# dusk-network/dusk-blindbidproof

Hardware: AMD Instinct MI355X
Metric: blind-bid proofs/sec (higher is better)
Workload: dtype u32

## Files before the change

### dusk_blindbidproof_amd/csrc/msm.hip

```cpp
#include "context.h"

namespace bbp {

#ifndef BBP_FOLD_PRIO
#define BBP_FOLD_PRIO 2
#endif
#ifndef BBP_MSM_WAVES
#define BBP_MSM_WAVES 2
#endif
#ifndef BBP_MSM_WAVES_MAX
#define BBP_MSM_WAVES_MAX 2
#endif

#ifdef BBP_MSM_PROF
__device__ unsigned long long g_msm_prof[8];
#define MSM_PROF_BEGIN() unsigned long long prof_t = wall_clock64()
#define MSM_PROF_MARK(i)                                                    \
    if (tid == 0) {                                                         \
        unsigned long long now_ = wall_clock64();                           \
        atomicAdd(&g_msm_prof[i], now_ - prof_t);                           \
        prof_t = now_;                                                      \
    }
#else
#define MSM_PROF_BEGIN()
// ... 11 lines not shown

__device__ __forceinline__ void xch_put(u32* xch, const ge& p) {
    const u32* w = reinterpret_cast<const u32*>(&p);
#pragma unroll
    for (int i = 0; i < GE_WORDS; i++) xch[i] = w[i];
}

__device__ __forceinline__ ge xch_get(const u32* xch) {
    ge p;
    u32* w = reinterpret_cast<u32*>(&p);
#pragma unroll
    for (int i = 0; i < GE_WORDS; i++) w[i] = xch[i];
    return p;
}

__device__ __forceinline__ row_regs load_row(const niels_row* __restrict__ tab, u32 entry, u32* __restrict__ fault) {
    u32 row = entry & 0x7fffffffu;
    if (row > (u32)(TAB_BASES * MSM_POS - 1)) {
        row = (u32)(TAB_BASES * MSM_POS - 1);
        atomicOr(fault, 1u);
    }
#ifdef BBP_EXP_ROWMASK
    row &= BBP_EXP_ROWMASK;
#endif
    return load_row_at(tab + row, entry >> 31);
}

#ifdef BBP_ACC_COOP
constexpr int COOP_IMG = 64 * 128;
__device__ __forceinline__ u32 coop_clamp_row(u32 entry, u32* __restrict__ fault) {
    u32 row = entry & 0x7fffffffu;
    if (row > (u32)(TAB_BASES * MSM_POS - 1)) {
        row = (u32)(TAB_BASES * MSM_POS - 1);
        atomicOr(fault, 1u);
    }
    return row;
}
__device__ __forceinline__ void coop_issue(const niels_row* __restrict__ tab, u8* wb, u32 my_row, int lane, u32 srcoff) {
    const u8* t = reinterpret_cast<const u8*>(tab);
    u32 r[8];
#pragma unroll
    for (int j = 0; j < 8; j++) r[j] = (u32)__shfl((int)my_row, 8 * j + (lane >> 3), 64);
#pragma unroll
    for (int j = 0; j < 8; j++) {
        const u8* src = t + (size_t)r[j] * 128 + (srcoff ^ (u32)((j & 1) << 6));
        __builtin_amdgcn_global_load_lds((const __attribute__((address_space(1))) void*)src, (__attribute__((address_space(3))) void*)(wb + j * 1024), 16, 0, 0);
    }
}
__device__ __forceinline__ row_regs coop_read(const u8* wb, u32 A, u32 neg) {
    const u32 An = A ^ (neg << 6);
    const uint4 a0 = *reinterpret_cast<const uint4*>(wb + An), a1 = *reinterpret_cast<const uint4*>(wb + (An ^ 0x10u));
    const uint2 a2 = *reinterpret_cast<const uint2*>(wb + (An ^ 0x20u));
    const uint4 b0 = *reinterpret_cast<const uint4*>(wb + (An ^ 0x40u)), b1 = *reinterpret_cast<const uint4*>(wb + (An ^ 0x50u));
    const uint2 b2 = *reinterpret_cast<const uint2*>(wb + (An ^ 0x60u));
    const uint2 x0 = *reinterpret_cast<const uint2*>(wb + (A ^ 0x20u) + 8);
    const uint4 x1 = *reinterpret_cast<const uint4*>(wb + (A ^ 0x30u));
    const uint2 x2 = *reinterpret_cast<const uint2*>(wb + (A ^ 0x60u) + 8), x3 = *reinterpret_cast<const uint2*>(wb + (A ^ 0x70u));
    row_regs r;
    r.ypx = fe{{(i32)a0.x, (i32)a0.y, (i32)a0.z, (i32)a0.w, (i32)a1.x, (i32)a1.y, (i32)a1.z, (i32)a1.w, (i32)a2.x, (i32)a2.y}};
    r.ymx = fe{{(i32)b0.x, (i32)b0.y, (i32)b0.z, (i32)b0.w, (i32)b1.x, (i32)b1.y, (i32)b1.z, (i32)b1.w, (i32)b2.x, (i32)b2.y}};
    r.xy2d = fe{{(i32)x0.x, (i32)x0.y, (i32)x1.x, (i32)x1.y, (i32)x1.z, (i32)x1.w, (i32)x2.x, (i32)x2.y, (i32)x3.x, (i32)x3.y}};
    return r;
}
#endif

__device__ __noinline__ void ge_add_nc(ge& r, const ge& a, const ge& b) { r = ge_add(a, b); }
__device__ __noinline__ void ge_dbl_nc(ge& r, const ge& a) { r = ge_dbl(a); }

#ifndef BBP_SORT_T
#define BBP_SORT_T 1024
#endif
constexpr int SORT_T = BBP_SORT_T;
template <int MODE> struct msm_geom;
template <> struct msm_geom<0> { static constexpr int K = MSM_K, NAF = MSM_NAF, W = MSM_W; };
template <> struct msm_geom<1> { static constexpr int K = FOLD_K, NAF = FOLD_NAF, W = FOLD_W; };
template <> struct msm_geom<2> { static constexpr int K = SMALL_K, NAF = SMALL_NAF, W = SMALL_W; };

template <int MODE>
__global__ __launch_bounds__(SORT_T) void k_msm_sort(const u32* __restrict__ scal_a, const u32* __restrict__ aux, u32 n_total, u32 n_idx_sets,
                                                      u32 n_sub, u32 split, u32* __restrict__ sorted_all, u32* __restrict__ cursor_all,
                                                      const u32* __restrict__ msm_map, const u32* __restrict__ n_active, u32* __restrict__ ticket) {
    constexpr int K = msm_geom<MODE>::K, NAF = msm_geom<MODE>::NAF, W = msm_geom<MODE>::W, G = K >= SORT_T ? K / SORT_T : 1;
    __shared__ u32 cursor[K + 1];
    __shared__ u32 part[SORT_T];
    const int tid = threadIdx.x;
    if (ticket && blockIdx.x == 0 && tid == 0) *ticket = 0;
    if (n_active && blockIdx.x >= *n_active) return;
    const size_t work = blockIdx.x, msm = work / split;
    const u32 i0 = (u32)(work % split) * n_sub;
    const u32 n = i0 < n_total ? min(n_sub, n_total - i0) : 0u;
    __builtin_amdgcn_s_setprio(3);
    const u32* sbase;
    const u32* base_idx = nullptr;
    u32 base0 = 0;
    if (MODE != 1) {
        const size_t src = msm_map ? (size_t)msm_map[msm] : msm;
        sbase = scal_a + (src * (size_t)n_total + i0) * 8;
        base_idx = aux + (size_t)(msm % n_idx_sets) * n_total + i0;
    } else {
        const u32 side = (u32)msm & 1u;
        sbase = (side ? aux : scal_a) + ((msm >> 1) * (size_t)2048 + i0) * 8;
        base0 = (side ? BBP_BASE_H0 : BBP_BASE_G0) + i0;
    }
    u32* sorted = sorted_all + work * (size_t)n_sub * W;
    auto key = [&](u32 i, u32 mag) -> u32 { return (MODE != 1 ? 0u : ((i0 + i) & (FOLD_CLS - 1)) * FOLD_M) + ((mag + 1) >> 1); };

    for (int k = tid; k <= K; k += SORT_T) cursor[k] = 0;
    __syncthreads();
    for (u32 i = tid; i < n; i += SORT_T) {
        const uint4* sp = reinterpret_cast<const uint4*>(sbase + (size_t)i * 8);
        uint4 lo = sp[0], hi = sp[1];
        const u32 s[8] = {lo.x, lo.y, lo.z, lo.w, hi.x, hi.y, hi.z, hi.w};
        if (MODE != 1 && base_idx[i] == MSM_SKIP_BASE) continue;
        sc_for_each_naf_digit<NAF>(s, [&](u32, u32 mag, u32) { atomicAdd(&cursor[key(i, mag)], 1u); });
    }
    __syncthreads();
    {
        u32 local = 0;
        for (int r = 1; r <= G; r++)
            if (tid * G + r <= K) local += cursor[tid * G + r];
        const int lane = tid & 63, wave = tid >> 6;
        u32 incl = local;
#pragma unroll
        for (int d = 1; d < 64; d <<= 1) {
            const u32 up = (u32)__shfl_up((int)incl, d, 64);
            if (lane >= d) incl += up;
        }
        if (lane == 63) part[wave] = incl;
        __syncthreads();
        if (tid < 64) {
            constexpr int NW = SORT_T / 64;
            u32 v = tid < NW ? part[tid] : 0u, sc_ = v;
#pragma unroll
            for (int d = 1; d < 64; d <<= 1) {
                const u32 up = (u32)__shfl_up((int)sc_, d, 64);
                if (tid >= d) sc_ += up;
            }
            if (tid < NW) part[tid] = sc_ - v;
        }
        __syncthreads();
        u32 base = part[wave] + incl - local;
        for (int r = 1; r <= G; r++) {
            if (tid * G + r > K) break;
            const u32 c = cursor[tid * G + r];
            cursor[tid * G + r] = base;
            base += c;
        }
    }
    __syncthreads();
    for (u32 i = tid; i < n; i += SORT_T) {
        const uint4* sp = reinterpret_cast<const uint4*>(sbase + (size_t)i * 8);
        uint4 lo = sp[0], hi = sp[1];
        const u32 s[8] = {lo.x, lo.y, lo.z, lo.w, hi.x, hi.y, hi.z, hi.w};
        if (MODE != 1 && base_idx[i] == MSM_SKIP_BASE) continue;
        const u32 tb = (MODE != 1 ? base_idx[i] : base0 + i) * MSM_POS;
        sc_for_each_naf_digit<NAF>(s, [&](u32 pos, u32 mag, u32 neg) {
            u32 at = atomicAdd(&cursor[key(i, mag)], 1u);
            sorted[at] = (tb + pos) | (neg << 31);
        });
    }
    __syncthreads();
    u32* cur_out = cursor_all + work * (size_t)(K + 1);
    for (int k = tid; k <= K; k += SORT_T) cur_out[k] = k ? cursor[k] : 0u;
}

#ifndef BBP_SORT_CAP
#define BBP_SORT_CAP 21504
#endif
template <int MODE> struct sort_cap { static constexpr u32 V = BBP_SORT_CAP; };
template <> struct sort_cap<1> { static constexpr u32 V = 8192; };
constexpr u32 SORT_CAP_WIDE = 32768;
constexpr u32 SORT_WIDE_FROM = 3000;

template <int MODE>
__global__ __launch_bounds__(SORT_T) void k_msm_sort_staged(const u32* __restrict__ scal_a, const u32* __restrict__ aux, u32 n_total, u32 n_idx_sets,
                                                             u32 n_sub, u32 split, u32* __restrict__ sorted_all, u32* __restrict__ cursor_all,
                                                             const u32* __restrict__ msm_map, const u32* __restrict__ n_active, u32 CAP, u32* __restrict__ ticket) {
    constexpr int K = msm_geom<MODE>::K, NAF = msm_geom<MODE>::NAF, W = msm_geom<MODE>::W, G = K >= SORT_T ? K / SORT_T : 1;
    extern __shared__ u32 stage[];
    __shared__ u32 start[K + 2];
    __shared__ u32 fill[K + 1];
    __shared__ u32 part[SORT_T];
    const int tid = threadIdx.x;
    if (ticket && blockIdx.x == 0 && tid == 0) *ticket = 0;
    if (n_active && blockIdx.x >= *n_active) return;
    const size_t work = blockIdx.x, msm = work / split;
    const u32 i0 = (u32)(work % split) * n_sub;
    const u32 n = i0 < n_total ? min(n_sub, n_total - i0) : 0u;
    __builtin_amdgcn_s_setprio(3);
    const u32* sbase;
    const u32* base_idx = nullptr;
    u32 base0 = 0;
    if (MODE != 1) {
        const size_t src = msm_map ? (size_t)msm_map[msm] : msm;
        sbase = scal_a + (src * (size_t)n_total + i0) * 8;
        base_idx = aux + (size_t)(msm % n_idx_sets) * n_total + i0;
    } else {
        const u32 side = (u32)msm & 1u;
        sbase = (side ? aux : scal_a) + ((msm >> 1) * (size_t)2048 + i0) * 8;
        base0 = (side ? BBP_BASE_H0 : BBP_BASE_G0) + i0;
    }
    u32* sorted = sorted_all + work * (size_t)n_sub * W;
    auto key = [&](u32 i, u32 mag) -> u32 { return (MODE != 1 ? 0u : ((i0 + i) & (FOLD_CLS - 1)) * FOLD_M) + ((mag + 1) >> 1); };

    for (int k = tid; k <= K; k += SORT_T) fill[k] = 0;
    __syncthreads();
    for (u32 i = tid; i < n; i += SORT_T) {
        const uint4* sp = reinterpret_cast<const uint4*>(sbase + (size_t)i * 8);
        uint4 lo = sp[0], hi = sp[1];
        const u32 s[8] = {lo.x, lo.y, lo.z, lo.w, hi.x, hi.y, hi.z, hi.w};
        if (MODE != 1 && base_idx[i] == MSM_SKIP_BASE) continue;
        sc_for_each_naf_digit<NAF>(s, [&](u32, u32 mag, u32) { atomicAdd(&fill[key(i, mag)], 1u); });
    }
    __syncthreads();
    {
        u32 local = 0;
        for (int r = 1; r <= G; r++)
            if (tid * G + r <= K) local += fill[tid * G + r];
        const int lane = tid & 63, wave = tid >> 6;
        u32 incl = local;
#pragma unroll
        for (int d = 1; d < 64; d <<= 1) {
            const u32 up = (u32)__shfl_up((int)incl, d, 64);
            if (lane >= d) incl += up;
        }
        if (lane == 63) part[wave] = incl;
        __syncthreads();
        if (tid < 64) {
            constexpr int NW = SORT_T / 64;
            u32 v = tid < NW ? part[tid] : 0u, sc_ = v;
#pragma unroll
            for (int d = 1; d < 64; d <<= 1) {
                const u32 up = (u32)__shfl_up((int)sc_, d, 64);
                if (tid >= d) sc_ += up;
            }
            if (tid < NW) part[tid] = sc_ - v;
        }
        __syncthreads();
        u32 base = part[wave] + incl - local;
        for (int r = 1; r <= G; r++) {
            if (tid * G + r > K) break;
            const u32 c = fill[tid * G + r];
            start[tid * G + r] = base;
            fill[tid * G + r] = 0;
            base += c;
        }
        if (tid == SORT_T - 1) start[K + 1] = base;
        if (tid == 0) start[0] = 0;
    }
    __syncthreads();
    u32 kb = 1;
    while (kb <= (u32)K) {
        const u32 base = start[kb];
        const bool direct = start[kb + 1] - base > CAP;
        u32 ke = kb + 1;
        if (!direct) {
            u32 lo = kb + 1, hi = (u32)K + 1;
            while (lo < hi) {
                const u32 mid = (lo + hi + 1) >> 1;
                if (start[mid] - base <= CAP) lo = mid; else hi = mid - 1;
            }
            ke = lo;
        }
        if (start[ke] != base) {
            for (u32 i = tid; i < n; i += SORT_T) {
                const uint4* sp = reinterpret_cast<const uint4*>(sbase + (size_t)i * 8);
                uint4 lo4 = sp[0], hi4 = sp[1];
                const u32 s[8] = {lo4.x, lo4.y, lo4.z, lo4.w, hi4.x, hi4.y, hi4.z, hi4.w};
                if (MODE != 1 && base_idx[i] == MSM_SKIP_BASE) continue;
                const u32 tb = (MODE != 1 ? base_idx[i] : base0 + i) * MSM_POS;
                sc_for_each_naf_digit<NAF>(s, [&](u32 pos, u32 mag, u32 neg) {
                    const u32 k = key(i, mag);
                    if (k >= kb && k < ke) {
                        const u32 at = start[k] + atomicAdd(&fill[k], 1u);
                        const u32 ent = (tb + pos) | (neg << 31);
                        if (direct) sorted[at] = ent; else stage[at - base] = ent;
                    }
                });
            }
            __syncthreads();
            if (!direct) {
                const u32 cnt = start[ke] - base;
                for (u32 i = tid; i < cnt; i += SORT_T) sorted[base + i] = stage[i];
            }
            __syncthreads();
        }
        kb = ke;
    }
    u32* cur_out = cursor_all + work * (size_t)(K + 1);
    for (int k = tid; k <= K; k += SORT_T) cur_out[k] = k ? start[k + 1] : 0u;
}

#ifndef BBP_ACC_WG
#define BBP_ACC_WG 256
#endif
constexpr int ACC_WG = BBP_ACC_WG, ACC_WGS = ACC_T / ACC_WG;
static_assert(ACC_T % ACC_WG == 0 && ACC_WG % 64 == 0, "accumulate workgroup geometry");

template <int MODE>
__global__ __launch_bounds__(ACC_WG) __attribute__((amdgpu_waves_per_eu(BBP_MSM_WAVES, BBP_MSM_WAVES_MAX)))
void k_msm_acc(const niels_row* __restrict__ ptable, const u32* __restrict__ sorted_all, const u32* __restrict__ cursor_all, u32 n ,
               ge* __restrict__ bsum_all, ge* __restrict__ psum_all, ge* __restrict__ out, const u32* __restrict__ n_active, u32* __restrict__ fault,
               u32 n_work, u32* __restrict__ ticket) {
    constexpr int K = msm_geom<MODE>::K, W = msm_geom<MODE>::W, G = K / MSM_T;
    __shared__ u32 cursor[K + 1];
#ifdef BBP_ACC_PERSIST
    static_assert(ACC_WGS == 1, "the persistent form draws whole MSMs");
    __shared__ u32 s_ticket;
  for (;;) {
    __syncthreads();
    if (threadIdx.x == 0) s_ticket = atomicAdd(ticket, 1u);
    __syncthreads();
    const size_t msm = s_ticket;
    if (msm >= n_work || (n_active && msm >= *n_active)) return;
    const int tid = (int)threadIdx.x;
#else
    const size_t msm = blockIdx.x / ACC_WGS;
    const int tid = (int)(blockIdx.x % ACC_WGS) * ACC_WG + (int)threadIdx.x;
    if (n_active && msm >= *n_active) return;
#endif
    const u32* sorted = sorted_all + msm * (size_t)n * W;
#ifdef BBP_MSM_PRIO
    __builtin_amdgcn_s_setprio(BBP_MSM_PRIO);
#endif
    MSM_PROF_BEGIN();
    {
        const u32* cur_in = cursor_all + msm * (size_t)(K + 1);
        for (int k = threadIdx.x; k <= K; k += ACC_WG) cursor[k] = cur_in[k];
    }
    __syncthreads();
    MSM_PROF_MARK(1);

    const u32 E = cursor[K];
    ge* bsum = bsum_all + msm * (size_t)K;
    ge* psum = psum_all + msm * (size_t)ACC_T;
#ifdef BBP_KO_ACC_PERMILLE
    const u32 c0 = (u32)(((u64)tid * E) / ACC_T), c1 = c0 + (u32)(((u64)((u32)(((u64)(tid + 1) * E) / ACC_T) - c0) * BBP_KO_ACC_PERMILLE) / 1000);
#else
    const u32 c0 = (u32)(((u64)tid * E) / ACC_T), c1 = (u32)(((u64)(tid + 1) * E) / ACC_T);
#endif
#ifdef BBP_MSM_PROF
    const unsigned long long clk0 = clock64();
#endif
    u32 k_first = 0;
    bool inside = false;
#ifdef BBP_ACC_COOP
    {
        __shared__ __attribute__((aligned(1024))) u8 rowimg[ACC_WG / 64][COOP_IMG];
        const int lane = (int)threadIdx.x & 63;
        u8* wb = rowimg[threadIdx.x >> 6];
        const u32 A = (u32)lane * 128u + ((((u32)lane >> 1) & 7u) << 4);
        const u32 srcoff = (((u32)lane & 7u) ^ (((u32)lane >> 3) >> 1)) << 4;
        const u32 n_it = (E + (u32)ACC_T - 1) / (u32)ACC_T, len = c1 - c0;
        u32 k = 1, kend = 0;
        ge* dest = &psum[tid];
        if (len) {
            u32 lo = 1, hi = K;
            while (lo < hi) {
                u32 mid = (lo + hi) >> 1;
                if (cursor[mid] > c0) hi = mid; else lo = mid + 1;
            }
            k = lo, kend = cursor[k];
            k_first = lo;
            inside = cursor[k - 1] < c0;
            if (!inside) dest = &bsum[k - 1];
        }
        ge acc = ge_identity();
        u32 ent_cur = len ? sorted[c0] : 0u;
        u32 ent_nxt = len > 1 ? sorted[c0 + 1] : 0u;
        if (n_it) coop_issue(ptable, wb, coop_clamp_row(ent_cur, fault), lane, srcoff);
        for (u32 it = 0; it < n_it; it++) {
            const u32 e = c0 + it;
            const row_regs cur = coop_read(wb, A, ent_cur >> 31);
            const bool neg = ent_cur >> 31;
            ent_cur = ent_nxt;
            const bool live = it < len;
            if (live && e == kend) {
                *dest = acc;
                acc = ge_identity();
                do { k++; kend = cursor[k]; } while (kend == e);
                dest = &bsum[k - 1];
            }
            asm volatile("s_waitcnt lgkmcnt(0)" ::: "memory");
            if (it + 1 < n_it) coop_issue(ptable, wb, coop_clamp_row(ent_cur, fault), lane, srcoff);
            if (it + 2 < len) ent_nxt = sorted[e + 2]; else ent_nxt = 0u;
            if (live) acc = ge_madd_row(acc, cur, neg);
        }
        if (len) *dest = acc;
    }
#else
    if (c0 < c1) {
        u32 lo = 1, hi = K;
        while (lo < hi) {
            u32 mid = (lo + hi) >> 1;
            if (cursor[mid] > c0) hi = mid; else lo = mid + 1;
        }
        u32 k = lo, kend = cursor[k];
        k_first = lo;
        inside = cursor[k - 1] < c0;
        ge* dest = inside ? &psum[tid] : &bsum[k - 1];
        ge acc = ge_identity();
        u32 ent_cur = sorted[c0];
        u32 ent_nxt = (c0 + 1 < c1) ? sorted[c0 + 1] : 0u;
        row_regs row = load_row(ptable, ent_cur, fault);
        for (u32 e = c0; e < c1; e++) {
            if (e == kend) {
                *dest = acc;
                acc = ge_identity();
                do { k++; kend = cursor[k]; } while (kend == e);
                dest = &bsum[k - 1];
            }
            const row_regs cur = row;
            const bool neg = ent_cur >> 31;
            ent_cur = ent_nxt;
            if (e + 1 < c1) row = load_row(ptable, ent_cur, fault);
            if (e + 2 < c1) ent_nxt = sorted[e + 2];
            acc = ge_madd_row(acc, cur, neg);
        }
        *dest = acc;
    }
#endif
#ifdef BBP_MSM_PROF
    if (tid == 0) atomicAdd(&g_msm_prof[6], clock64() - clk0);
#endif
    MSM_PROF_MARK(2);
    __threadfence_block();
    __syncthreads();
    MSM_PROF_MARK(3);
#ifdef BBP_ACC_PERSIST
  }
#endif
}

template <int MODE>
__global__ __launch_bounds__(MSM_T) void k_msm_fold(const u32* __restrict__ cursor_all, ge* __restrict__ bsum_all, const ge* __restrict__ psum_all,
                                                     ge* __restrict__ out, const u32* __restrict__ n_active) {
    constexpr int K = msm_geom<MODE>::K, G = K / MSM_T;
    __shared__ u32 cursor[K + 1];
    __shared__ u32 xch[GE_WORDS];
    const int tid = threadIdx.x;
    if (n_active && blockIdx.x >= *n_active) return;
    __builtin_amdgcn_s_setprio(BBP_FOLD_PRIO);
    const size_t msm = blockIdx.x;
    {
        const u32* cur_in = cursor_all + msm * (size_t)(K + 1);
        for (int k = tid; k <= K; k += MSM_T) cursor[k] = cur_in[k];
// ... 292 lines not shown
    }
    if (o < n_out && j == 0) out[o] = acc;
}

static u32 msm_split(u32 n_msm, u32 n_terms) {
    static const u32 below = [] { const char* e = getenv("BBP_MSM_SPLIT_BELOW"); return e ? (u32)atoi(e) : 128u; }();
    static const u32 target = [] { const char* e = getenv("BBP_MSM_SPLIT_TARGET"); return e ? (u32)atoi(e) : 512u; }();
    if (n_msm >= below) return 1;
    u32 s = target / n_msm;
    if (s > 16) s = 16;
    while (s > 1 && n_terms / s < 128) s--;
    return s ? s : 1;
}

struct MsmScratch {
    u32 *sorted, *cursor;
    ge *bsum, *psum, *tmp;
    u32* ticket;
    size_t bytes;
};
static MsmScratch msm_scratch_layout(void* base, size_t n_msm, size_t n_terms, size_t W, size_t K, size_t out_items = 1) {
    auto up = [](size_t x) { return (x + 255) / 256 * 256; };
    MsmScratch m;
    size_t o = 0;
    m.sorted = reinterpret_cast<u32*>(static_cast<u8*>(base) + o);
    o += up(n_msm * n_terms * W * sizeof(u32));
    m.cursor = reinterpret_cast<u32*>(static_cast<u8*>(base) + o);
    o += up(n_msm * (K + 1) * sizeof(u32));
    m.bsum = reinterpret_cast<ge*>(static_cast<u8*>(base) + o);
    o += n_msm * K * sizeof(ge);
    m.psum = reinterpret_cast<ge*>(static_cast<u8*>(base) + o);
    o += n_msm * ACC_T * sizeof(ge);
    m.tmp = reinterpret_cast<ge*>(static_cast<u8*>(base) + o);
    o += up(n_msm * out_items * sizeof(ge));
    m.ticket = reinterpret_cast<u32*>(static_cast<u8*>(base) + o);
    o += 256;
    m.bytes = o;
    return m;
}
size_t msm_scratch_bytes(uint32_t n_msm, uint32_t n_terms) {
    const u32 split = msm_split(n_msm, n_terms), n_sub = (n_terms + split - 1) / split;
    size_t a = msm_scratch_layout(nullptr, (size_t)n_msm * split, n_sub, MSM_W, MSM_K).bytes;
    if (split > 1) a = std::max(a, msm_scratch_layout(nullptr, (size_t)n_msm * split, n_sub, SMALL_W, SMALL_K).bytes);
    const size_t b = msm_scratch_layout(nullptr, n_msm, n_terms, MSM_W, MSM_K).bytes;
    return a > b ? a : b;
}

static inline u32 acc_grid(bbp_ctx*, u32 n_work) {
#ifdef BBP_ACC_PERSIST
    static const u32 cap = [] { const char* e = getenv("BBP_ACC_PERSIST_GRID"); return e ? (u32)atoi(e) : 512u; }();
    return n_work < cap ? n_work : cap;
#else
    return n_work * ACC_WGS;
#endif
}

int32_t fold_generators_launch(bbp_ctx* ctx, uint32_t n_proofs, const sc* g_dev, const sc* h_dev, ge* out_dev, hipStream_t stream,
                               int scratch_slot) {
    if (n_proofs == 0) return BBP_OK;
    const size_t n_msm = 2 * (size_t)n_proofs;
    const u32 split = msm_split((u32)n_msm, 2048), n_sub = (2048 + split - 1) / split;
    const size_t n_work = n_msm * split;
    DevBuf& scratch = ctx->slice_fold[scratch_slot];
    int32_t rc = dev_reserve(ctx, scratch, msm_scratch_layout(nullptr, n_work, n_sub, FOLD_W, FOLD_K, FOLD_CLS).bytes);
    if (rc) return rc;
    const MsmScratch m = msm_scratch_layout(scratch.p, n_work, n_sub, FOLD_W, FOLD_K, FOLD_CLS);
    {
        ScopedEvent ev(ctx, TAG_MSM_SORT, stream);
        if (ctx->sort_staged & 2) {
            if (!ctx->sort_lds_attr1) {
                BBP_HIP_TRY(ctx, hipFuncSetAttribute((const void*)k_msm_sort_staged<1>, hipFuncAttributeMaxDynamicSharedMemorySize, (int)(sort_cap<1>::V * 4)));
                ctx->sort_lds_attr1 = true;
            }
            hipLaunchKernelGGL(k_msm_sort_staged<1>, dim3((u32)n_work), dim3(SORT_T), sort_cap<1>::V * 4, stream, (const u32*)g_dev, (const u32*)h_dev, 2048u, 1u,
                               n_sub, split, m.sorted, m.cursor, (const u32*)nullptr, (const u32*)nullptr, sort_cap<1>::V, m.ticket);
        } else
            hipLaunchKernelGGL(k_msm_sort<1>, dim3((u32)n_work), dim3(SORT_T), 0, stream, (const u32*)g_dev, (const u32*)h_dev, 2048u, 1u, n_sub, split,
                               m.sorted, m.cursor, (const u32*)nullptr, (const u32*)nullptr, m.ticket);
        BBP_HIP_TRY(ctx, hipGetLastError());
    }
    {
        ScopedEvent ev(ctx, TAG_MSM, stream);
        hipLaunchKernelGGL(k_msm_acc<1>, dim3(acc_grid(ctx, (u32)n_work)), dim3(ACC_WG), 0, stream, ctx->ptable, m.sorted, m.cursor, n_sub, m.bsum, m.psum,
                           split > 1 ? m.tmp : out_dev, (const u32*)nullptr, ctx->health, (u32)n_work, m.ticket);
        BBP_HIP_TRY(ctx, hipGetLastError());
    }
    ScopedEvent evf(ctx, TAG_MSM_FOLD, stream);
    hipLaunchKernelGGL(k_msm_fold<1>, dim3((u32)n_work), dim3(MSM_T), 0, stream, m.cursor, m.bsum, m.psum, split > 1 ? m.tmp : out_dev,
                       (const u32*)nullptr);
    BBP_HIP_TRY(ctx, hipGetLastError());
    if (split > 1) {
        const u32 n_out = (u32)n_msm * FOLD_CLS;
        hipLaunchKernelGGL(k_msm_reduce, dim3((n_out * REDUCE_L + 63) / 64), dim3(64), lds_token(ctx), stream, n_out, split, (u32)FOLD_CLS, m.tmp, out_dev);
        BBP_HIP_TRY(ctx, hipGetLastError());
    }
    return BBP_OK;
}

__global__ __launch_bounds__(64) void k_encode(const ge* __restrict__ pts, u32 n, u32* __restrict__ out_words) {
// ... 15 lines not shown
    if (n_msm == 0) return BBP_OK;
    if (n_terms == 0 || n_terms > 65535u) {
        ctx->err = "msm_launch: n_terms out of range";
        return BBP_ERR_BAD_ARG;
    }
    DevBuf& scratch = scratch_slot ? ctx->slice_sorted[scratch_slot] : ctx->sorted;
    int32_t rc = dev_reserve(ctx, scratch, msm_scratch_bytes(n_msm, n_terms));
    if (rc) return rc;
    const u32 split = n_active_dev ? 1u : msm_split(n_msm, n_terms), n_sub = (n_terms + split - 1) / split;
    const u32 n_work = n_msm * split;
    if (split > 1 && ctx->msm_small) {
        const MsmScratch ms = msm_scratch_layout(scratch.p, n_work, n_sub, SMALL_W, SMALL_K);
        {
            ScopedEvent ev(ctx, TAG_MSM_SORT, stream);
            hipLaunchKernelGGL(k_msm_sort<2>, dim3(n_work), dim3(SORT_T), 0, stream, scalars_dev, base_idx_dev, n_terms, n_idx_sets, n_sub, split, ms.sorted, ms.cursor,
                               msm_map_dev, n_active_dev, ms.ticket);
            BBP_HIP_TRY(ctx, hipGetLastError());
        }
        if (ctx->debug_corrupt) {
            ctx->debug_corrupt = 0;
            hipLaunchKernelGGL(k_debug_poke, dim3(1), dim3(1), 0, stream, ms.sorted);
            BBP_HIP_TRY(ctx, hipGetLastError());
        }
        {
            ScopedEvent ev(ctx, TAG_MSM, stream);
            hipLaunchKernelGGL(k_msm_acc<2>, dim3(acc_grid(ctx, n_work)), dim3(ACC_WG), 0, stream, ctx->ptable, ms.sorted, ms.cursor, n_sub, ms.bsum, ms.psum, ms.tmp,
                               n_active_dev, ctx->health, n_work, ms.ticket);
            BBP_HIP_TRY(ctx, hipGetLastError());
        }
        {
            ScopedEvent evf(ctx, TAG_MSM_FOLD, stream);
            hipLaunchKernelGGL(k_msm_fold<2>, dim3(n_work), dim3(MSM_T), 0, stream, ms.cursor, ms.bsum, ms.psum, ms.tmp, n_active_dev);
            BBP_HIP_TRY(ctx, hipGetLastError());
        }
        hipLaunchKernelGGL(k_msm_reduce, dim3((n_msm * REDUCE_L + 63) / 64), dim3(64), lds_token(ctx), stream, n_msm, split, 1u, ms.tmp, out_points_dev);
        BBP_HIP_TRY(ctx, hipGetLastError());
        return BBP_OK;
    }
    const MsmScratch m = msm_scratch_layout(scratch.p, n_work, n_sub, MSM_W, MSM_K);
    {
        ScopedEvent ev(ctx, TAG_MSM_SORT, stream);
        const bool wide = n_sub > SORT_WIDE_FROM;
        if ((ctx->sort_staged & 1) && (!wide || (ctx->sort_staged & 4))) {
            const u32 cap = wide ? SORT_CAP_WIDE : sort_cap<0>::V;
            if (!ctx->sort_lds_attr) {
                BBP_HIP_TRY(ctx, hipFuncSetAttribute((const void*)k_msm_sort_staged<0>, hipFuncAttributeMaxDynamicSharedMemorySize, (int)(SORT_CAP_WIDE * 4)));
                ctx->sort_lds_attr = true;
            }
            hipLaunchKernelGGL(k_msm_sort_staged<0>, dim3(n_work), dim3(SORT_T), cap * 4, stream, scalars_dev, base_idx_dev, n_terms, n_idx_sets, n_sub, split,
                               m.sorted, m.cursor, msm_map_dev, n_active_dev, cap, m.ticket);
        }
        else
            hipLaunchKernelGGL(k_msm_sort<0>, dim3(n_work), dim3(SORT_T), 0, stream, scalars_dev, base_idx_dev, n_terms, n_idx_sets, n_sub, split,
                               m.sorted, m.cursor, msm_map_dev, n_active_dev, m.ticket);
        BBP_HIP_TRY(ctx, hipGetLastError());
    }
    if (ctx->debug_corrupt) {
        ctx->debug_corrupt = 0;
        hipLaunchKernelGGL(k_debug_poke, dim3(1), dim3(1), 0, stream, m.sorted);
        BBP_HIP_TRY(ctx, hipGetLastError());
    }
    chain_acc = chain_acc && ctx->verify_serial_acc;
    if (chain_acc && ctx->vacc_valid)
        BBP_HIP_TRY(ctx, hipStreamWaitEvent(stream, ctx->ev_vacc[ctx->vacc_seq % bbp_ctx::VACC_RING], 0));
    {
        ScopedEvent ev(ctx, TAG_MSM, stream);
        hipLaunchKernelGGL(k_msm_acc<0>, dim3(acc_grid(ctx, n_work)), dim3(ACC_WG), 0, stream, ctx->ptable, m.sorted, m.cursor, n_sub, m.bsum, m.psum,
                           split > 1 ? m.tmp : out_points_dev, n_active_dev, ctx->health, n_work, m.ticket);
        BBP_HIP_TRY(ctx, hipGetLastError());
    }
    static const bool chain_after_fold = getenv("BBP_VERIFY_CHAIN_AFTER_FOLD") && atoi(getenv("BBP_VERIFY_CHAIN_AFTER_FOLD"));
    if (chain_acc && !chain_after_fold) {
        ctx->vacc_seq++;
        BBP_HIP_TRY(ctx, hipEventRecord(ctx->ev_vacc[ctx->vacc_seq % bbp_ctx::VACC_RING], stream));
        ctx->vacc_valid = true;
    }
    ScopedEvent evf(ctx, TAG_MSM_FOLD, stream);
    if (n_work >= (u32)ctx->fold_half_from)
        hipLaunchKernelGGL(k_msm_fold_half, dim3((n_work + 1) / 2), dim3(64), 0, stream, m.cursor, m.bsum, m.psum, split > 1 ? m.tmp : out_points_dev,
                           n_work, n_active_dev);
    else
        hipLaunchKernelGGL(k_msm_fold<0>, dim3(n_work), dim3(MSM_T), 0, stream, m.cursor, m.bsum, m.psum, split > 1 ? m.tmp : out_points_dev, n_active_dev);
    BBP_HIP_TRY(ctx, hipGetLastError());
// ... 32 lines not shown
```

### dusk_blindbidproof_amd/csrc/point.h

```cpp
#pragma once
#include "field.h"

namespace bbp {

struct ge {
    fe X, Y, Z, T;
};

struct ge_niels {
    fe ypx, ymx, xy2d;
};

struct niels_packed {
    u32 w[24];
};

struct alignas(128) niels_row {
    i32 v[32];
};

BBP_HD niels_packed niels_pack(const ge_niels& n) {
    niels_packed p;
    fe_towords(p.w, n.ypx);
    fe_towords(p.w + 8, n.ymx);
// ... 133 lines not shown
}

__device__ __forceinline__ ge ge_madd_row(const ge& p, const row_regs& q, bool neg) {
    fe a = fe_mul(fe_sub(p.Y, p.X), q.ymx);
    fe b = fe_mul(fe_add(p.Y, p.X), q.ypx);
    fe c = fe_mul(p.T, q.xy2d);
    fe d = fe_add(p.Z, p.Z);
    fe e = fe_sub(b, a), h = fe_add(b, a);
    fe f0 = fe_sub(d, c), g0 = fe_add(d, c);
    fe f = fe_select(f0, g0, neg), g = fe_select(g0, f0, neg);
    ge r;
    r.X = fe_mul(e, f);
    r.Y = fe_mul(g, h);
    r.Z = fe_mul(g, f);
    r.T = fe_mul(e, h);
    return r;
}
#endif

BBP_HD ge_niels ge_to_niels(const ge& p, const fe& zinv) {
    fe x = fe_mul(p.X, zinv), y = fe_mul(p.Y, zinv);
    ge_niels r;
    r.ypx = fe_add(y, x);
    r.ymx = fe_sub(y, x);
    r.xy2d = fe_mul(fe_mul(x, y), fe_d2());
    return r;
}

BBP_HD ge ge_from_niels(const ge_niels& n) {
    const fe half = BBP_FE_LIT(0xfffffff7u, 0xffffffffu, 0xffffffffu, 0xffffffffu, 0xffffffffu, 0xffffffffu, 0xffffffffu, 0x3fffffffu);
// ... 96 lines not shown
```

Before: 21450.

## Split MSM buckets by sign so accumulation skips per-point negation

The sort kernels now bucket entries by sign as well as magnitude and emit a per-bucket boundary (cpos) between the negative and positive runs. The accumulation kernel adds the negative run first, negates the partial sum once, then continues with the positives. This removes the per-entry conditional negation from the mixed-add inner loop. Row loads become plain 8x uint4 loads with an asm wait anchor and a sched_barrier in the madd. The unused cooperative-LDS and persistent-ticket paths are dropped, and the extra scratch array costs more memory traffic in the sort.

```diff
diff --git a/dusk_blindbidproof_amd/csrc/msm.hip b/dusk_blindbidproof_amd/csrc/msm.hip
--- a/dusk_blindbidproof_amd/csrc/msm.hip
+++ b/dusk_blindbidproof_amd/csrc/msm.hip
@@ -49,8 +49,11 @@
     return p;
 }
 
-__device__ __forceinline__ row_regs load_row(const niels_row* __restrict__ tab, u32 entry, u32* __restrict__ fault) {
-    u32 row = entry & 0x7fffffffu;
+struct row_fetch {
+    row_regs r;
+    u32 pad0, pad1;
+};
+__device__ __forceinline__ row_fetch load_row(const niels_row* __restrict__ tab, u32 row, u32* __restrict__ fault) {
     if (row > (u32)(TAB_BASES * MSM_POS - 1)) {
         row = (u32)(TAB_BASES * MSM_POS - 1);
         atomicOr(fault, 1u);
@@ -58,46 +61,16 @@
 #ifdef BBP_EXP_ROWMASK
     row &= BBP_EXP_ROWMASK;
 #endif
-    return load_row_at(tab + row, entry >> 31);
-}
-
-#ifdef BBP_ACC_COOP
-constexpr int COOP_IMG = 64 * 128;
-__device__ __forceinline__ u32 coop_clamp_row(u32 entry, u32* __restrict__ fault) {
-    u32 row = entry & 0x7fffffffu;
-    if (row > (u32)(TAB_BASES * MSM_POS - 1)) {
-        row = (u32)(TAB_BASES * MSM_POS - 1);
-        atomicOr(fault, 1u);
-    }
-    return row;
-}
-__device__ __forceinline__ void coop_issue(const niels_row* __restrict__ tab, u8* wb, u32 my_row, int lane, u32 srcoff) {
-    const u8* t = reinterpret_cast<const u8*>(tab);
-    u32 r[8];
-#pragma unroll
-    for (int j = 0; j < 8; j++) r[j] = (u32)__shfl((int)my_row, 8 * j + (lane >> 3), 64);
-#pragma unroll
-    for (int j = 0; j < 8; j++) {
-        const u8* src = t + (size_t)r[j] * 128 + (srcoff ^ (u32)((j & 1) << 6));
-        __builtin_amdgcn_global_load_lds((const __attribute__((address_space(1))) void*)src, (__attribute__((address_space(3))) void*)(wb + j * 1024), 16, 0, 0);
-    }
-}
-__device__ __forceinline__ row_regs coop_read(const u8* wb, u32 A, u32 neg) {
-    const u32 An = A ^ (neg << 6);
-    const uint4 a0 = *reinterpret_cast<const uint4*>(wb + An), a1 = *reinterpret_cast<const uint4*>(wb + (An ^ 0x10u));
-    const uint2 a2 = *reinterpret_cast<const uint2*>(wb + (An ^ 0x20u));
-    const uint4 b0 = *reinterpret_cast<const uint4*>(wb + (An ^ 0x40u)), b1 = *reinterpret_cast<const uint4*>(wb + (An ^ 0x50u));
-    const uint2 b2 = *reinterpret_cast<const uint2*>(wb + (An ^ 0x60u));
-    const uint2 x0 = *reinterpret_cast<const uint2*>(wb + (A ^ 0x20u) + 8);
-    const uint4 x1 = *reinterpret_cast<const uint4*>(wb + (A ^ 0x30u));
-    const uint2 x2 = *reinterpret_cast<const uint2*>(wb + (A ^ 0x60u) + 8), x3 = *reinterpret_cast<const uint2*>(wb + (A ^ 0x70u));
-    row_regs r;
-    r.ypx = fe{{(i32)a0.x, (i32)a0.y, (i32)a0.z, (i32)a0.w, (i32)a1.x, (i32)a1.y, (i32)a1.z, (i32)a1.w, (i32)a2.x, (i32)a2.y}};
-    r.ymx = fe{{(i32)b0.x, (i32)b0.y, (i32)b0.z, (i32)b0.w, (i32)b1.x, (i32)b1.y, (i32)b1.z, (i32)b1.w, (i32)b2.x, (i32)b2.y}};
-    r.xy2d = fe{{(i32)x0.x, (i32)x0.y, (i32)x1.x, (i32)x1.y, (i32)x1.z, (i32)x1.w, (i32)x2.x, (i32)x2.y, (i32)x3.x, (i32)x3.y}};
-    return r;
-}
-#endif
+    const uint4* q = reinterpret_cast<const uint4*>(tab + row);
+    const uint4 w0 = q[0], w1 = q[1], w2 = q[2], w3 = q[3], w4 = q[4], w5 = q[5], w6 = q[6], w7 = q[7];
+    row_fetch f;
+    f.r.ypx = fe{{(i32)w0.x, (i32)w0.y, (i32)w0.z, (i32)w0.w, (i32)w1.x, (i32)w1.y, (i32)w1.z, (i32)w1.w, (i32)w2.x, (i32)w2.y}};
+    f.r.ymx = fe{{(i32)w4.x, (i32)w4.y, (i32)w4.z, (i32)w4.w, (i32)w5.x, (i32)w5.y, (i32)w5.z, (i32)w5.w, (i32)w6.x, (i32)w6.y}};
+    f.r.xy2d = fe{{(i32)w2.z, (i32)w2.w, (i32)w3.x, (i32)w3.y, (i32)w3.z, (i32)w3.w, (i32)w6.z, (i32)w6.w, (i32)w7.x, (i32)w7.y}};
+    f.pad0 = w7.z, f.pad1 = w7.w;
+    return f;
+}
+__device__ __forceinline__ void row_landed(const row_fetch& f) { asm volatile("" ::"v"(f.pad0), "v"(f.pad1)); }
 
 __device__ __noinline__ void ge_add_nc(ge& r, const ge& a, const ge& b) { r = ge_add(a, b); }
 __device__ __noinline__ void ge_dbl_nc(ge& r, const ge& a) { r = ge_dbl(a); }
@@ -114,12 +87,11 @@
 template <int MODE>
 __global__ __launch_bounds__(SORT_T) void k_msm_sort(const u32* __restrict__ scal_a, const u32* __restrict__ aux, u32 n_total, u32 n_idx_sets,
                                                       u32 n_sub, u32 split, u32* __restrict__ sorted_all, u32* __restrict__ cursor_all,
-                                                      const u32* __restrict__ msm_map, const u32* __restrict__ n_active, u32* __restrict__ ticket) {
+                                                      u32* __restrict__ cpos_all, const u32* __restrict__ msm_map, const u32* __restrict__ n_active) {
     constexpr int K = msm_geom<MODE>::K, NAF = msm_geom<MODE>::NAF, W = msm_geom<MODE>::W, G = K >= SORT_T ? K / SORT_T : 1;
-    __shared__ u32 cursor[K + 1];
+    __shared__ u32 cursor[2 * (K + 1)];
     __shared__ u32 part[SORT_T];
     const int tid = threadIdx.x;
-    if (ticket && blockIdx.x == 0 && tid == 0) *ticket = 0;
     if (n_active && blockIdx.x >= *n_active) return;
     const size_t work = blockIdx.x, msm = work / split;
     const u32 i0 = (u32)(work % split) * n_sub;
@@ -140,20 +112,20 @@
     u32* sorted = sorted_all + work * (size_t)n_sub * W;
     auto key = [&](u32 i, u32 mag) -> u32 { return (MODE != 1 ? 0u : ((i0 + i) & (FOLD_CLS - 1)) * FOLD_M) + ((mag + 1) >> 1); };
 
-    for (int k = tid; k <= K; k += SORT_T) cursor[k] = 0;
+    for (int k = tid; k < 2 * (K + 1); k += SORT_T) cursor[k] = 0;
     __syncthreads();
     for (u32 i = tid; i < n; i += SORT_T) {
         const uint4* sp = reinterpret_cast<const uint4*>(sbase + (size_t)i * 8);
         uint4 lo = sp[0], hi = sp[1];
         const u32 s[8] = {lo.x, lo.y, lo.z, lo.w, hi.x, hi.y, hi.z, hi.w};
         if (MODE != 1 && base_idx[i] == MSM_SKIP_BASE) continue;
-        sc_for_each_naf_digit<NAF>(s, [&](u32, u32 mag, u32) { atomicAdd(&cursor[key(i, mag)], 1u); });
+        sc_for_each_naf_digit<NAF>(s, [&](u32, u32 mag, u32 neg) { atomicAdd(&cursor[2 * key(i, mag) + (neg ^ 1u)], 1u); });
     }
     __syncthreads();
     {
         u32 local = 0;
         for (int r = 1; r <= G; r++)
-            if (tid * G + r <= K) local += cursor[tid * G + r];
+            if (tid * G + r <= K) local += cursor[2 * (tid * G + r)] + cursor[2 * (tid * G + r) + 1];
         const int lane = tid & 63, wave = tid >> 6;
         u32 incl = local;
 #pragma unroll
@@ -177,9 +149,10 @@
         u32 base = part[wave] + incl - local;
         for (int r = 1; r <= G; r++) {
             if (tid * G + r > K) break;
-            const u32 c = cursor[tid * G + r];
-            cursor[tid * G + r] = base;
-            base += c;
+            const u32 cn = cursor[2 * (tid * G + r)], cp = cursor[2 * (tid * G + r) + 1];
+            cursor[2 * (tid * G + r)] = base;
+            cursor[2 * (tid * G + r) + 1] = base + cn;
+            base += cn + cp;
         }
     }
     __syncthreads();
@@ -190,13 +163,17 @@
         if (MODE != 1 && base_idx[i] == MSM_SKIP_BASE) continue;
         const u32 tb = (MODE != 1 ? base_idx[i] : base0 + i) * MSM_POS;
         sc_for_each_naf_digit<NAF>(s, [&](u32 pos, u32 mag, u32 neg) {
-            u32 at = atomicAdd(&cursor[key(i, mag)], 1u);
-            sorted[at] = (tb + pos) | (neg << 31);
+            u32 at = atomicAdd(&cursor[2 * key(i, mag) + (neg ^ 1u)], 1u);
+            sorted[at] = tb + pos;
         });
     }
     __syncthreads();
     u32* cur_out = cursor_all + work * (size_t)(K + 1);
-    for (int k = tid; k <= K; k += SORT_T) cur_out[k] = k ? cursor[k] : 0u;
+    u32* cpos_out = cpos_all + work * (size_t)(K + 1);
+    for (int k = tid; k <= K; k += SORT_T) {
+        cur_out[k] = k ? cursor[2 * k + 1] : 0u;
+        cpos_out[k] = k ? cursor[2 * k] : 0u;
+    }
 }
 
 #ifndef BBP_SORT_CAP
@@ -210,14 +187,25 @@
 template <int MODE>
 __global__ __launch_bounds__(SORT_T) void k_msm_sort_staged(const u32* __restrict__ scal_a, const u32* __restrict__ aux, u32 n_total, u32 n_idx_sets,
                                                              u32 n_sub, u32 split, u32* __restrict__ sorted_all, u32* __restrict__ cursor_all,
-                                                             const u32* __restrict__ msm_map, const u32* __restrict__ n_active, u32 CAP, u32* __restrict__ ticket) {
+                                                             u32* __restrict__ cpos_all, const u32* __restrict__ msm_map, const u32* __restrict__ n_active, u32 CAP) {
     constexpr int K = msm_geom<MODE>::K, NAF = msm_geom<MODE>::NAF, W = msm_geom<MODE>::W, G = K >= SORT_T ? K / SORT_T : 1;
     extern __shared__ u32 stage[];
     __shared__ u32 start[K + 2];
-    __shared__ u32 fill[K + 1];
+    constexpr bool PACK = MODE == 1;
+    static_assert(!PACK || (2048 / FOLD_CLS) * FOLD_W < 65536, "a composite bucket's entry count must fit a half-word");
+    constexpr int NF = PACK ? K + 1 : 2 * (K + 1);
+    __shared__ u32 fill[NF];
     __shared__ u32 part[SORT_T];
     const int tid = threadIdx.x;
-    if (ticket && blockIdx.x == 0 && tid == 0) *ticket = 0;
+    auto bump = [&](u32 k, u32 neg) -> u32 {
+        if (PACK) {
+            const u32 o = atomicAdd(&fill[k], neg ? 1u : 0x10000u);
+            return neg ? (o & 0xffffu) : (o >> 16);
+        }
+        return atomicAdd(&fill[2 * k + (neg ^ 1u)], 1u);
+    };
+    auto cnt_neg = [&](u32 k) -> u32 { return PACK ? (fill[k] & 0xffffu) : fill[2 * k]; };
+    auto cnt_pos = [&](u32 k) -> u32 { return PACK ? (fill[k] >> 16) : fill[2 * k + 1]; };
     if (n_active && blockIdx.x >= *n_active) return;
     const size_t work = blockIdx.x, msm = work / split;
     const u32 i0 = (u32)(work % split) * n_sub;
@@ -238,20 +226,20 @@
     u32* sorted = sorted_all + work * (size_t)n_sub * W;
     auto key = [&](u32 i, u32 mag) -> u32 { return (MODE != 1 ? 0u : ((i0 + i) & (FOLD_CLS - 1)) * FOLD_M) + ((mag + 1) >> 1); };
 
-    for (int k = tid; k <= K; k += SORT_T) fill[k] = 0;
+    for (int k = tid; k < NF; k += SORT_T) fill[k] = 0;
     __syncthreads();
     for (u32 i = tid; i < n; i += SORT_T) {
         const uint4* sp = reinterpret_cast<const uint4*>(sbase + (size_t)i * 8);
         uint4 lo = sp[0], hi = sp[1];
         const u32 s[8] = {lo.x, lo.y, lo.z, lo.w, hi.x, hi.y, hi.z, hi.w};
         if (MODE != 1 && base_idx[i] == MSM_SKIP_BASE) continue;
-        sc_for_each_naf_digit<NAF>(s, [&](u32, u32 mag, u32) { atomicAdd(&fill[key(i, mag)], 1u); });
+        sc_for_each_naf_digit<NAF>(s, [&](u32, u32 mag, u32 neg) { bump(key(i, mag), neg); });
     }
     __syncthreads();
     {
         u32 local = 0;
         for (int r = 1; r <= G; r++)
-            if (tid * G + r <= K) local += fill[tid * G + r];
+            if (tid * G + r <= K) local += cnt_neg(tid * G + r) + cnt_pos(tid * G + r);
         const int lane = tid & 63, wave = tid >> 6;
         u32 incl = local;
 #pragma unroll
@@ -275,10 +263,10 @@
         u32 base = part[wave] + incl - local;
         for (int r = 1; r <= G; r++) {
             if (tid * G + r > K) break;
-            const u32 c = fill[tid * G + r];
-            start[tid * G + r] = base;
-            fill[tid * G + r] = 0;
-            base += c;
+            const u32 k = tid * G + r, cn = cnt_neg(k), cp = cnt_pos(k);
+            start[k] = base;
+            if constexpr (PACK) fill[k] = cn << 16; else fill[2 * k] = 0, fill[2 * k + 1] = cn;
+            base += cn + cp;
         }
         if (tid == SORT_T - 1) start[K + 1] = base;
         if (tid == 0) start[0] = 0;
@@ -307,8 +295,8 @@
                 sc_for_each_naf_digit<NAF>(s, [&](u32 pos, u32 mag, u32 neg) {
                     const u32 k = key(i, mag);
                     if (k >= kb && k < ke) {
-                        const u32 at = start[k] + atomicAdd(&fill[k], 1u);
-                        const u32 ent = (tb + pos) | (neg << 31);
+                        const u32 at = start[k] + bump(k, neg);
+                        const u32 ent = tb + pos;
                         if (direct) sorted[at] = ent; else stage[at - base] = ent;
                     }
                 });
@@ -323,7 +311,11 @@
         kb = ke;
     }
     u32* cur_out = cursor_all + work * (size_t)(K + 1);
-    for (int k = tid; k <= K; k += SORT_T) cur_out[k] = k ? start[k + 1] : 0u;
+    u32* cpos_out = cpos_all + work * (size_t)(K + 1);
+    for (int k = tid; k <= K; k += SORT_T) {
+        cur_out[k] = k ? start[k + 1] : 0u;
+        cpos_out[k] = k ? start[k] + cnt_neg(k) : 0u;
+    }
 }
 
 #ifndef BBP_ACC_WG
@@ -334,26 +326,14 @@
 
 template <int MODE>
 __global__ __launch_bounds__(ACC_WG) __attribute__((amdgpu_waves_per_eu(BBP_MSM_WAVES, BBP_MSM_WAVES_MAX)))
-void k_msm_acc(const niels_row* __restrict__ ptable, const u32* __restrict__ sorted_all, const u32* __restrict__ cursor_all, u32 n ,
-               ge* __restrict__ bsum_all, ge* __restrict__ psum_all, ge* __restrict__ out, const u32* __restrict__ n_active, u32* __restrict__ fault,
-               u32 n_work, u32* __restrict__ ticket) {
-    constexpr int K = msm_geom<MODE>::K, W = msm_geom<MODE>::W, G = K / MSM_T;
+void k_msm_acc(const niels_row* __restrict__ ptable, const u32* __restrict__ sorted_all, const u32* __restrict__ cursor_all, const u32* __restrict__ cpos_all,
+               u32 n , ge* __restrict__ bsum_all, ge* __restrict__ psum_all, const u32* __restrict__ n_active, u32* __restrict__ fault) {
+    constexpr int K = msm_geom<MODE>::K, W = msm_geom<MODE>::W;
     __shared__ u32 cursor[K + 1];
-#ifdef BBP_ACC_PERSIST
-    static_assert(ACC_WGS == 1, "the persistent form draws whole MSMs");
-    __shared__ u32 s_ticket;
-  for (;;) {
-    __syncthreads();
-    if (threadIdx.x == 0) s_ticket = atomicAdd(ticket, 1u);
-    __syncthreads();
-    const size_t msm = s_ticket;
-    if (msm >= n_work || (n_active && msm >= *n_active)) return;
-    const int tid = (int)threadIdx.x;
-#else
+    __shared__ u32 cpos[K + 1];
     const size_t msm = blockIdx.x / ACC_WGS;
     const int tid = (int)(blockIdx.x % ACC_WGS) * ACC_WG + (int)threadIdx.x;
     if (n_active && msm >= *n_active) return;
-#endif
     const u32* sorted = sorted_all + msm * (size_t)n * W;
 #ifdef BBP_MSM_PRIO
     __builtin_amdgcn_s_setprio(BBP_MSM_PRIO);
@@ -361,7 +341,8 @@
     MSM_PROF_BEGIN();
     {
         const u32* cur_in = cursor_all + msm * (size_t)(K + 1);
-        for (int k = threadIdx.x; k <= K; k += ACC_WG) cursor[k] = cur_in[k];
+        const u32* pos_in = cpos_all + msm * (size_t)(K + 1);
+        for (int k = threadIdx.x; k <= K; k += ACC_WG) cursor[k] = cur_in[k], cpos[k] = pos_in[k];
     }
     __syncthreads();
     MSM_PROF_MARK(1);
@@ -377,53 +358,6 @@
 #ifdef BBP_MSM_PROF
     const unsigned long long clk0 = clock64();
 #endif
-    u32 k_first = 0;
-    bool inside = false;
-#ifdef BBP_ACC_COOP
-    {
-        __shared__ __attribute__((aligned(1024))) u8 rowimg[ACC_WG / 64][COOP_IMG];
-        const int lane = (int)threadIdx.x & 63;
-        u8* wb = rowimg[threadIdx.x >> 6];
-        const u32 A = (u32)lane * 128u + ((((u32)lane >> 1) & 7u) << 4);
-        const u32 srcoff = (((u32)lane & 7u) ^ (((u32)lane >> 3) >> 1)) << 4;
-        const u32 n_it = (E + (u32)ACC_T - 1) / (u32)ACC_T, len = c1 - c0;
-        u32 k = 1, kend = 0;
-        ge* dest = &psum[tid];
-        if (len) {
-            u32 lo = 1, hi = K;
-            while (lo < hi) {
-                u32 mid = (lo + hi) >> 1;
-                if (cursor[mid] > c0) hi = mid; else lo = mid + 1;
-            }
-            k = lo, kend = cursor[k];
-            k_first = lo;
-            inside = cursor[k - 1] < c0;
-            if (!inside) dest = &bsum[k - 1];
-        }
-        ge acc = ge_identity();
-        u32 ent_cur = len ? sorted[c0] : 0u;
-        u32 ent_nxt = len > 1 ? sorted[c0 + 1] : 0u;
-        if (n_it) coop_issue(ptable, wb, coop_clamp_row(ent_cur, fault), lane, srcoff);
-        for (u32 it = 0; it < n_it; it++) {
-            const u32 e = c0 + it;
-            const row_regs cur = coop_read(wb, A, ent_cur >> 31);
-            const bool neg = ent_cur >> 31;
-            ent_cur = ent_nxt;
-            const bool live = it < len;
-            if (live && e == kend) {
-                *dest = acc;
-                acc = ge_identity();
-                do { k++; kend = cursor[k]; } while (kend == e);
-                dest = &bsum[k - 1];
-            }
-            asm volatile("s_waitcnt lgkmcnt(0)" ::: "memory");
-            if (it + 1 < n_it) coop_issue(ptable, wb, coop_clamp_row(ent_cur, fault), lane, srcoff);
-            if (it + 2 < len) ent_nxt = sorted[e + 2]; else ent_nxt = 0u;
-            if (live) acc = ge_madd_row(acc, cur, neg);
-        }
-        if (len) *dest = acc;
-    }
-#else
     if (c0 < c1) {
         u32 lo = 1, hi = K;
         while (lo < hi) {
@@ -431,30 +365,34 @@
             if (cursor[mid] > c0) hi = mid; else lo = mid + 1;
         }
         u32 k = lo, kend = cursor[k];
-        k_first = lo;
-        inside = cursor[k - 1] < c0;
-        ge* dest = inside ? &psum[tid] : &bsum[k - 1];
+        ge* dest = cursor[k - 1] < c0 ? &psum[tid] : &bsum[k - 1];
+        bool negd = c0 < cpos[k];
+        u32 nxt = negd ? cpos[k] : kend;
         ge acc = ge_identity();
-        u32 ent_cur = sorted[c0];
         u32 ent_nxt = (c0 + 1 < c1) ? sorted[c0 + 1] : 0u;
-        row_regs row = load_row(ptable, ent_cur, fault);
+        row_fetch row = load_row(ptable, sorted[c0], fault);
         for (u32 e = c0; e < c1; e++) {
-            if (e == kend) {
-                *dest = acc;
-                acc = ge_identity();
-                do { k++; kend = cursor[k]; } while (kend == e);
-                dest = &bsum[k - 1];
-            }
-            const row_regs cur = row;
-            const bool neg = ent_cur >> 31;
-            ent_cur = ent_nxt;
-            if (e + 1 < c1) row = load_row(ptable, ent_cur, fault);
+            if (e == nxt) {
+                if (negd) acc = ge_neg(acc);
+                negd = false;
+                if (e == kend) {
+                    *dest = acc;
+                    acc = ge_identity();
+                    do { k++; kend = cursor[k]; } while (kend == e);
+                    dest = &bsum[k - 1];
+                    negd = e < cpos[k];
+                }
+                nxt = negd ? cpos[k] : kend;
+            }
+            row_landed(row);
+            const row_regs cur = row.r;
+            if (e + 1 < c1) row = load_row(ptable, ent_nxt, fault);
             if (e + 2 < c1) ent_nxt = sorted[e + 2];
-            acc = ge_madd_row(acc, cur, neg);
-        }
+            acc = ge_madd_row(acc, cur);
+        }
+        if (negd) acc = ge_neg(acc);
         *dest = acc;
     }
-#endif
 #ifdef BBP_MSM_PROF
     if (tid == 0) atomicAdd(&g_msm_prof[6], clock64() - clk0);
 #endif
@@ -462,9 +400,6 @@
     __threadfence_block();
     __syncthreads();
     MSM_PROF_MARK(3);
-#ifdef BBP_ACC_PERSIST
-  }
-#endif
 }
 
 template <int MODE>
@@ -787,9 +722,8 @@
 }
 
 struct MsmScratch {
-    u32 *sorted, *cursor;
+    u32 *sorted, *cursor, *cpos;
     ge *bsum, *psum, *tmp;
-    u32* ticket;
     size_t bytes;
 };
 static MsmScratch msm_scratch_layout(void* base, size_t n_msm, size_t n_terms, size_t W, size_t K, size_t out_items = 1) {
@@ -800,14 +734,14 @@
     o += up(n_msm * n_terms * W * sizeof(u32));
     m.cursor = reinterpret_cast<u32*>(static_cast<u8*>(base) + o);
     o += up(n_msm * (K + 1) * sizeof(u32));
+    m.cpos = reinterpret_cast<u32*>(static_cast<u8*>(base) + o);
+    o += up(n_msm * (K + 1) * sizeof(u32));
     m.bsum = reinterpret_cast<ge*>(static_cast<u8*>(base) + o);
     o += n_msm * K * sizeof(ge);
     m.psum = reinterpret_cast<ge*>(static_cast<u8*>(base) + o);
     o += n_msm * ACC_T * sizeof(ge);
     m.tmp = reinterpret_cast<ge*>(static_cast<u8*>(base) + o);
     o += up(n_msm * out_items * sizeof(ge));
-    m.ticket = reinterpret_cast<u32*>(static_cast<u8*>(base) + o);
-    o += 256;
     m.bytes = o;
     return m;
 }
@@ -817,15 +751,6 @@
     if (split > 1) a = std::max(a, msm_scratch_layout(nullptr, (size_t)n_msm * split, n_sub, SMALL_W, SMALL_K).bytes);
     const size_t b = msm_scratch_layout(nullptr, n_msm, n_terms, MSM_W, MSM_K).bytes;
     return a > b ? a : b;
-}
-
-static inline u32 acc_grid(bbp_ctx*, u32 n_work) {
-#ifdef BBP_ACC_PERSIST
-    static const u32 cap = [] { const char* e = getenv("BBP_ACC_PERSIST_GRID"); return e ? (u32)atoi(e) : 512u; }();
-    return n_work < cap ? n_work : cap;
-#else
-    return n_work * ACC_WGS;
-#endif
 }
 
 int32_t fold_generators_launch(bbp_ctx* ctx, uint32_t n_proofs, const sc* g_dev, const sc* h_dev, ge* out_dev, hipStream_t stream,
@@ -846,16 +771,16 @@
                 ctx->sort_lds_attr1 = true;
             }
             hipLaunchKernelGGL(k_msm_sort_staged<1>, dim3((u32)n_work), dim3(SORT_T), sort_cap<1>::V * 4, stream, (const u32*)g_dev, (const u32*)h_dev, 2048u, 1u,
-                               n_sub, split, m.sorted, m.cursor, (const u32*)nullptr, (const u32*)nullptr, sort_cap<1>::V, m.ticket);
+                               n_sub, split, m.sorted, m.cursor, m.cpos, (const u32*)nullptr, (const u32*)nullptr, sort_cap<1>::V);
         } else
             hipLaunchKernelGGL(k_msm_sort<1>, dim3((u32)n_work), dim3(SORT_T), 0, stream, (const u32*)g_dev, (const u32*)h_dev, 2048u, 1u, n_sub, split,
-                               m.sorted, m.cursor, (const u32*)nullptr, (const u32*)nullptr, m.ticket);
+                               m.sorted, m.cursor, m.cpos, (const u32*)nullptr, (const u32*)nullptr);
         BBP_HIP_TRY(ctx, hipGetLastError());
     }
     {
         ScopedEvent ev(ctx, TAG_MSM, stream);
-        hipLaunchKernelGGL(k_msm_acc<1>, dim3(acc_grid(ctx, (u32)n_work)), dim3(ACC_WG), 0, stream, ctx->ptable, m.sorted, m.cursor, n_sub, m.bsum, m.psum,
-                           split > 1 ? m.tmp : out_dev, (const u32*)nullptr, ctx->health, (u32)n_work, m.ticket);
+        hipLaunchKernelGGL(k_msm_acc<1>, dim3((u32)n_work * ACC_WGS), dim3(ACC_WG), 0, stream, ctx->ptable, m.sorted, m.cursor, m.cpos, n_sub, m.bsum, m.psum,
+                           (const u32*)nullptr, ctx->health);
         BBP_HIP_TRY(ctx, hipGetLastError());
     }
     ScopedEvent evf(ctx, TAG_MSM_FOLD, stream);
@@ -901,7 +826,7 @@
         {
             ScopedEvent ev(ctx, TAG_MSM_SORT, stream);
             hipLaunchKernelGGL(k_msm_sort<2>, dim3(n_work), dim3(SORT_T), 0, stream, scalars_dev, base_idx_dev, n_terms, n_idx_sets, n_sub, split, ms.sorted, ms.cursor,
-                               msm_map_dev, n_active_dev, ms.ticket);
+                               ms.cpos, msm_map_dev, n_active_dev);
             BBP_HIP_TRY(ctx, hipGetLastError());
         }
         if (ctx->debug_corrupt) {
@@ -911,8 +836,8 @@
         }
         {
             ScopedEvent ev(ctx, TAG_MSM, stream);
-            hipLaunchKernelGGL(k_msm_acc<2>, dim3(acc_grid(ctx, n_work)), dim3(ACC_WG), 0, stream, ctx->ptable, ms.sorted, ms.cursor, n_sub, ms.bsum, ms.psum, ms.tmp,
-                               n_active_dev, ctx->health, n_work, ms.ticket);
+            hipLaunchKernelGGL(k_msm_acc<2>, dim3(n_work * ACC_WGS), dim3(ACC_WG), 0, stream, ctx->ptable, ms.sorted, ms.cursor, ms.cpos, n_sub, ms.bsum, ms.psum,
+                               n_active_dev, ctx->health);
             BBP_HIP_TRY(ctx, hipGetLastError());
         }
         {
@@ -935,11 +860,11 @@
                 ctx->sort_lds_attr = true;
             }
             hipLaunchKernelGGL(k_msm_sort_staged<0>, dim3(n_work), dim3(SORT_T), cap * 4, stream, scalars_dev, base_idx_dev, n_terms, n_idx_sets, n_sub, split,
-                               m.sorted, m.cursor, msm_map_dev, n_active_dev, cap, m.ticket);
+                               m.sorted, m.cursor, m.cpos, msm_map_dev, n_active_dev, cap);
         }
         else
             hipLaunchKernelGGL(k_msm_sort<0>, dim3(n_work), dim3(SORT_T), 0, stream, scalars_dev, base_idx_dev, n_terms, n_idx_sets, n_sub, split,
-                               m.sorted, m.cursor, msm_map_dev, n_active_dev, m.ticket);
+                               m.sorted, m.cursor, m.cpos, msm_map_dev, n_active_dev);
         BBP_HIP_TRY(ctx, hipGetLastError());
     }
     if (ctx->debug_corrupt) {
@@ -952,8 +877,8 @@
         BBP_HIP_TRY(ctx, hipStreamWaitEvent(stream, ctx->ev_vacc[ctx->vacc_seq % bbp_ctx::VACC_RING], 0));
     {
         ScopedEvent ev(ctx, TAG_MSM, stream);
-        hipLaunchKernelGGL(k_msm_acc<0>, dim3(acc_grid(ctx, n_work)), dim3(ACC_WG), 0, stream, ctx->ptable, m.sorted, m.cursor, n_sub, m.bsum, m.psum,
-                           split > 1 ? m.tmp : out_points_dev, n_active_dev, ctx->health, n_work, m.ticket);
+        hipLaunchKernelGGL(k_msm_acc<0>, dim3(n_work * ACC_WGS), dim3(ACC_WG), 0, stream, ctx->ptable, m.sorted, m.cursor, m.cpos, n_sub, m.bsum, m.psum,
+                           n_active_dev, ctx->health);
         BBP_HIP_TRY(ctx, hipGetLastError());
     }
     static const bool chain_after_fold = getenv("BBP_VERIFY_CHAIN_AFTER_FOLD") && atoi(getenv("BBP_VERIFY_CHAIN_AFTER_FOLD"));
diff --git a/dusk_blindbidproof_amd/csrc/point.h b/dusk_blindbidproof_amd/csrc/point.h
--- a/dusk_blindbidproof_amd/csrc/point.h
+++ b/dusk_blindbidproof_amd/csrc/point.h
@@ -171,6 +171,21 @@
     r.Y = fe_mul(g, h);
     r.Z = fe_mul(g, f);
     r.T = fe_mul(e, h);
+    return r;
+}
+
+__device__ __forceinline__ ge ge_madd_row(const ge& p, const row_regs& q) {
+    fe a = fe_mul(fe_sub(p.Y, p.X), q.ymx);
+    fe b = fe_mul(fe_add(p.Y, p.X), q.ypx);
+    fe c = fe_mul(p.T, q.xy2d);
+    fe d = fe_add(p.Z, p.Z);
+    fe e = fe_sub(b, a), f = fe_sub(d, c), g = fe_add(d, c), h = fe_add(b, a);
+    ge r;
+    r.X = fe_mul(e, f);
+    r.T = fe_mul(e, h);
+    __builtin_amdgcn_sched_barrier(0);
+    r.Y = fe_mul(g, h);
+    r.Z = fe_mul(g, f);
     return r;
 }
 #endif
```

Result: no change. 21580 (median of 3 runs) (+0.6%).
